# Roboy/gym-roboy

Hardware: AMD Instinct MI355X
Metric: env-steps/sec, MsjRobot (3-DOF/8-tendon) batched rollout (higher is better)
Workload: dtype f32

## Files before the change

### gym_roboy_amd/csrc/gen_msj_baked.cpp

```cpp
#include <cstdio>
#include <string>

#include "msj_build.hpp"

extern "C" int rb_gen_msj_baked(const rb_robot_desc *d, double step_size, int nsub, const char *path) {
    rb::MsjConst<float, 8> c;
    std::string err;
    const int rc = rb::msj_build<float, 8>(d, step_size, nsub, &c, err);
    if (rc) return rc;
    FILE *f = std::fopen(path, "w");
    if (!f) return RB_EINVAL;
    std::fprintf(f, "// msj_baked.hpp - GENERATED by gen_msj_baked.cpp (tools/gen_msj_baked.py) from\n"
                    "// gym_roboy_amd/envs/robots/data/msj_platform.json: MsjRobot's closed-form constants as literals.\n"
                    "// Do not edit; regenerate.  Hex float literals: exact.\n#pragma once\n#include \"msj_math.hpp\"\n\nnamespace rbk {\n"
                    "#define RB_MSJ_BAKED_TABLE {{ \\\n");
    for (int k = 0; k < 8; ++k) {
        const auto &t = c.ten[k];
        std::fprintf(f, "  {{%af,%af,%af},{%af,%af,%af},{%af,%af,%af},%af,%af,%af,%af,%af,{0.0f,0.0f}}, \\\n", t.A[0], t.A[1], t.A[2],
                     t.Bv[0], t.Bv[1], t.Bv[2], t.B2[0], t.B2[1], t.B2[2], t.ab2, t.il0s, t.elcs, t.ksg, t.fmaxv);
    }
    std::fprintf(f, " }, {%af,%af,%af,%af,%af,%af}, {%af,%af,%af}, {%af,%af,%af}, \\\n", c.IO[0], c.IO[1], c.IO[2], c.IO[3], c.IO[4],
                 c.IO[5], c.mc[0], c.mc[1], c.mc[2], c.g[0], c.g[1], c.g[2]);
    std::fprintf(f, " {%af,%af,%af},{%af,%af,%af},{%af,%af,%af},{%af,%af,%af},{%af,%af,%af}, \\\n", c.arm[0], c.arm[1], c.arm[2],
                 c.damp[0], c.damp[1], c.damp[2], c.qlo[0], c.qlo[1], c.qlo[2], c.qhi[0], c.qhi[1], c.qhi[2], c.qdmax[0],
                 c.qdmax[1], c.qdmax[2]);
    std::fprintf(f, " %af,%af,%af,%af,%af,%af,%af,%af, %d,%d,%d}\n", c.kps, c.pe_k2s, c.inv_pe_den, c.fv_c1l, c.fv_c2l, c.fv_c2s,
                 c.fv_k, c.h, c.nsub, c.simple, c.nt);
    std::fprintf(f, "#if defined(__HIPCC__)\n__device__ constexpr rb::MsjConst<float, 8> BAKED = RB_MSJ_BAKED_TABLE;\n#endif\n"
                    "constexpr rb::MsjConst<float, 8> BAKED_HOST = RB_MSJ_BAKED_TABLE;\n}  // namespace rbk\n");
    std::fclose(f);
    return RB_OK;
}
```

### gym_roboy_amd/csrc/msj_baked.hpp

```cpp
#pragma once
#include "msj_math.hpp"

namespace rbk {
#define RB_MSJ_BAKED_TABLE {{ \
  {{0x1.5784fcp-4f,0x1.be2b16p-5f,-0x1.47ae14p-6f},{0x1.179142p-7f,0x1.48d0b8p-5f,0x1.b03512p-5f},{-0x1.dce646p-6f,-0x1.187458p-3f,-0x1.70a3d8p-3f},0x1.7f62b6p-6f,0x1.9090f6p+3f,-0x1.a30d8ap+0f,0x1.2c24dap+2f,0x1.99674ep+5f,{0.0f,0.0f}}, \
  {{0x1.be2b16p-5f,0x1.5784fcp-4f,-0x1.47ae14p-6f},{0x1.48d0b8p-5f,0x1.179142p-7f,0x1.b03512p-5f},{-0x1.187458p-3f,-0x1.dce646p-6f,-0x1.70a3d8p-3f},0x1.7f62b6p-6f,0x1.9090f6p+3f,-0x1.a30d8ap+0f,0x1.2c24dap+2f,0x1.99674ep+5f,{0.0f,0.0f}}, \
  {{-0x1.be2b16p-5f,0x1.5784fcp-4f,-0x1.47ae14p-6f},{-0x1.48d0b8p-5f,0x1.179142p-7f,0x1.b03512p-5f},{0x1.187458p-3f,-0x1.dce646p-6f,-0x1.70a3d8p-3f},0x1.7f62b6p-6f,0x1.9090f6p+3f,-0x1.a30d8ap+0f,0x1.2c24dap+2f,0x1.4785d8p+3f,{0.0f,0.0f}}, \
  {{-0x1.5784fcp-4f,0x1.be2b16p-5f,-0x1.47ae14p-6f},{-0x1.179142p-7f,0x1.48d0b8p-5f,0x1.b03512p-5f},{0x1.dce646p-6f,-0x1.187458p-3f,-0x1.70a3d8p-3f},0x1.7f62b6p-6f,0x1.9090f6p+3f,-0x1.a30d8ap+0f,0x1.2c24dap+2f,0x1.4785d8p+3f,{0.0f,0.0f}}, \
  {{-0x1.5784fcp-4f,-0x1.be2b16p-5f,-0x1.47ae14p-6f},{-0x1.179142p-7f,-0x1.48d0b8p-5f,0x1.b03512p-5f},{0x1.dce646p-6f,0x1.187458p-3f,-0x1.70a3d8p-3f},0x1.7f62b6p-6f,0x1.9090f6p+3f,-0x1.a30d8ap+0f,0x1.2c24dap+2f,0x1.4785d8p+3f,{0.0f,0.0f}}, \
  {{-0x1.be2b16p-5f,-0x1.5784fcp-4f,-0x1.47ae14p-6f},{-0x1.48d0b8p-5f,-0x1.179142p-7f,0x1.b03512p-5f},{0x1.187458p-3f,0x1.dce646p-6f,-0x1.70a3d8p-3f},0x1.7f62b6p-6f,0x1.9090f6p+3f,-0x1.a30d8ap+0f,0x1.2c24dap+2f,0x1.4785d8p+3f,{0.0f,0.0f}}, \
  {{0x1.be2b16p-5f,-0x1.5784fcp-4f,-0x1.47ae14p-6f},{0x1.48d0b8p-5f,-0x1.179142p-7f,0x1.b03512p-5f},{-0x1.187458p-3f,0x1.dce646p-6f,-0x1.70a3d8p-3f},0x1.7f62b6p-6f,0x1.9090f6p+3f,-0x1.a30d8ap+0f,0x1.2c24dap+2f,0x1.99674ep+5f,{0.0f,0.0f}}, \
  {{0x1.5784fcp-4f,-0x1.be2b16p-5f,-0x1.47ae14p-6f},{0x1.179142p-7f,-0x1.48d0b8p-5f,0x1.b03512p-5f},{-0x1.dce646p-6f,0x1.187458p-3f,-0x1.70a3d8p-3f},0x1.7f62b6p-6f,0x1.9090f6p+3f,-0x1.a30d8ap+0f,0x1.2c24dap+2f,0x1.99674ep+5f,{0.0f,0.0f}}, \
 }, {0x1.3a92a4p-10f,0x1.3a92a4p-10f,0x1.0624dep-11f,0x0p+0f,0x0p+0f,0x0p+0f}, {0x0p+0f,0x0p+0f,0x1.eb851ep-7f}, {0x0p+0f,0x0p+0f,-0x1.39eb86p+3f}, \
 {0x1.99999ap-3f,0x1.99999ap-3f,0x1.99999ap-3f},{0x1.99999ap-1f,0x1.99999ap-1f,0x1.99999ap-1f},{-0x1.ccccccp-2f,-0x1.ccccccp-2f,-0x1.333334p-1f},{0x1.ccccccp-2f,0x1.ccccccp-2f,0x1.333334p-1f},{0x1.0c1524p-1f,0x1.0c1524p-1f,0x1.0c1524p-1f}, \
 0x1.df8d2cp+1f,0x1.cd3b24p+1f,0x1.31aea4p-6f,0x1.ep+3f,0x1.4p+3f,-0x1p+2f,0x1.4p+2f,0x1.99999ap-4f, 1,1,8}
#if defined(__HIPCC__)
__device__ constexpr rb::MsjConst<float, 8> BAKED = RB_MSJ_BAKED_TABLE;
#endif
constexpr rb::MsjConst<float, 8> BAKED_HOST = RB_MSJ_BAKED_TABLE;
}
```

### gym_roboy_amd/csrc/msj_build.hpp

```cpp
#pragma once
#include <cmath>
#include <string>

#include "../../include/roboy_sim.h"
#include "msj_math.hpp"

namespace rb {

inline bool msj_class(const rb_robot_desc *d, std::string &why) {
    if (d->n_q != 3) { why = "n_q != 3"; return false; }
    for (int i = 0; i < 3; ++i) {
        if (d->parent[i] != i - 1) { why = "joints are not a serial chain"; return false; }
        for (int a = 0; a < 3; ++a) {
            if (d->origin[3 * i + a] != 0.0) { why = "joint origins are not co-located at the base origin"; return false; }
            if (std::fabs(d->axis[3 * i + a] - (a == i ? 1.0 : 0.0)) > 1e-12) { why = "joint axes are not x, y, z"; return false; }
        }
    }
    for (int i = 0; i < 2; ++i) {
        if (d->mass[i] != 0.0) { why = "virtual links 0/1 carry mass"; return false; }
        for (int a = 0; a < 6; ++a)
            if (d->inertia[6 * i + a] != 0.0) { why = "virtual links 0/1 carry inertia"; return false; }
    }
    for (int k = 0; k < d->n_t; ++k) {
        const int v0 = d->vp_offset[k], v1 = d->vp_offset[k + 1];
        if (v1 - v0 < 2) { why = "tendon with fewer than two via-points"; return false; }
        bool on_body = false;
        for (int v = v0; v < v1; ++v) {
            const int link = d->vp_link[v];
            if (link != -1 && link != 2) { why = "via-point on a virtual link"; return false; }
            if (link == 2) on_body = true;
            else if (on_body) { why = "tendon returns from the body to the base"; return false; }
        }
        if (d->vp_link[v0] != -1 || !on_body) { why = "tendon does not run base -> body"; return false; }
    }
    return true;
}

template <typename T, int NT>
int msj_build(const rb_robot_desc *d, double step_size, int nsub, MsjConst<T, NT> *out, std::string &err,
              bool exact = true) {
    if (!msj_class(d, err)) return RB_EUNSUPPORTED;
    if (exact ? d->n_t != NT : (d->n_t < 1 || d->n_t > NT)) {
        err = "tendon count does not match this kernel instance"; return RB_EUNSUPPORTED;
    }
    MsjConst<T, NT> &c = *out;
    const double log2e = 1.4426950408889634;
    const double sc = std::sqrt(log2e) / d->fl_width;
    auto seglen = [&](int va, int vb) {
        double s = 0.0;
        for (int a = 0; a < 3; ++a) { const double t = d->vp_pos[3 * vb + a] - d->vp_pos[3 * va + a]; s += t * t; }
        return std::sqrt(s);
    };
    for (int k = 0; k < d->n_t; ++k) {
        const int v0 = d->vp_offset[k], v1 = d->vp_offset[k + 1];
        int vb = v0;
        while (d->vp_link[vb] == -1) ++vb;
        const int va = vb - 1;
        double lc = 0.0;
        for (int v = v0; v + 1 < v1; ++v)
            if (v != va) lc += seglen(v, v + 1);
        const double moving0 = seglen(va, vb);
        if (moving0 < 1e-6) { err = "degenerate tendon segment"; return RB_EINVAL; }
        const double l0 = lc + moving0;
        MsjTendon<T> &t = c.ten[k];
        const double vl0 = d->v_max * l0;
        for (int a = 0; a < 3; ++a) { t.A[a] = T(d->vp_pos[3 * va + a]); t.Bv[a] = T(d->vp_pos[3 * vb + a] / vl0); }
        double ab2 = 0.0;
        for (int a = 0; a < 3; ++a) ab2 += d->vp_pos[3 * va + a] * d->vp_pos[3 * va + a] + d->vp_pos[3 * vb + a] * d->vp_pos[3 * vb + a];
        for (int a = 0; a < 3; ++a) t.B2[a] = T(-2.0 * d->vp_pos[3 * vb + a]);
        t.ab2 = T(ab2); t.il0s = T(sc / l0); t.elcs = T(sc * (lc / l0 - 1.0)); t.ksg = T(d->kp * d->setpoint_scale / l0);
        t.fmaxv = T(d->f_max[k] * vl0);
        t.pad[0] = t.pad[1] = T(0);
    }
    for (int k = d->n_t; k < NT; ++k) {
        MsjTendon<T> &t = c.ten[k];
        t.A[0] = T(1); t.A[1] = T(0); t.A[2] = T(0); t.Bv[0] = T(0); t.Bv[1] = T(0); t.Bv[2] = T(1);
        t.B2[0] = T(0); t.B2[1] = T(0); t.B2[2] = T(-2);
        t.ab2 = T(2); t.il0s = T(sc); t.elcs = T(-sc); t.ksg = T(0); t.fmaxv = T(0);
        t.pad[0] = t.pad[1] = T(0);
    }
    c.nt = d->n_t;
    const double m = d->mass[2];
    const double *cm = d->com + 6, *ic = d->inertia + 12;
    const double c2 = cm[0] * cm[0] + cm[1] * cm[1] + cm[2] * cm[2];
    c.IO[0] = T(ic[0] + m * (c2 - cm[0] * cm[0]));
    c.IO[1] = T(ic[1] + m * (c2 - cm[1] * cm[1]));
    c.IO[2] = T(ic[2] + m * (c2 - cm[2] * cm[2]));
    c.IO[3] = T(ic[3] - m * cm[0] * cm[1]);
    c.IO[4] = T(ic[4] - m * cm[0] * cm[2]);
    c.IO[5] = T(ic[5] - m * cm[1] * cm[2]);
    for (int a = 0; a < 3; ++a) {
        c.mc[a] = T(m * cm[a]);
        c.g[a] = T(d->gravity[a]);
        c.arm[a] = T(d->armature[a]); c.damp[a] = T(d->damping[a]);
        c.qlo[a] = T(d->q_lo[a]); c.qhi[a] = T(d->q_hi[a]); c.qdmax[a] = T(d->qd_max[a]);
    }
    c.kps = T(d->kp / sc);
    c.pe_k2s = T(log2e * d->kpe / (d->e0 * sc));
    c.inv_pe_den = T(1.0 / (std::exp(d->kpe) - 1.0));
    const double slope0 = 1.0 + 1.0 / d->fv_a;
    const double c2l = slope0 / (d->fv_n - 1.0);
    c.fv_c2s = T(-1.0 / d->fv_a);
    c.fv_k = T(1.0 + 1.0 / d->fv_a);
    c.fv_c1l = T(d->fv_n * c2l); c.fv_c2l = T(c2l);
    c.h = T(step_size / nsub); c.nsub = nsub;
    c.simple = (ic[3] == 0.0 && ic[4] == 0.0 && ic[5] == 0.0 && cm[0] == 0.0 && cm[1] == 0.0 &&
                d->gravity[0] == 0.0 && d->gravity[1] == 0.0) ? 1 : 0;
    return RB_OK;
}

template <typename T>
void msj_tendon_units(const rb_robot_desc *d, TendonUnits<T> *out, int nt_max) {
// ... 57 lines not shown
```

### gym_roboy_amd/csrc/msj_jit.hpp

```cpp
#pragma once
#include <dlfcn.h>
#include <hip/hip_runtime.h>
#include <hip/hiprtc.h>

#include <fcntl.h>
#include <sys/stat.h>
#include <unistd.h>

#include <atomic>
#include <cstdint>
#include <cstdio>
#include <cstdlib>
#include <cstring>
#include <string>
#include <vector>

#include "msj_math.hpp"

namespace rbj {

struct Module {
    hipModule_t mod = nullptr;
    hipFunction_t step[2] = {nullptr, nullptr};
    hipFunction_t env[2] = {nullptr, nullptr};
// ... 11 lines not shown
    decltype(&hiprtcGetCode) code = nullptr;
    decltype(&hiprtcDestroyProgram) destroy = nullptr;
    decltype(&hiprtcVersion) version = nullptr;
    bool ok = false;
};

inline const Rtc &rtc() {
    static Rtc r = [] {
        Rtc x;
        void *h = dlopen("libhiprtc.so", RTLD_NOW | RTLD_GLOBAL);
        if (!h) h = dlopen("/opt/rocm/lib/libhiprtc.so", RTLD_NOW | RTLD_GLOBAL);
        if (!h) return x;
#define RBJ_SYM(field, name) x.field = reinterpret_cast<decltype(x.field)>(dlsym(h, name))
        RBJ_SYM(create, "hiprtcCreateProgram"); RBJ_SYM(add_name, "hiprtcAddNameExpression");
        RBJ_SYM(compile, "hiprtcCompileProgram"); RBJ_SYM(log_size, "hiprtcGetProgramLogSize");
        RBJ_SYM(log, "hiprtcGetProgramLog"); RBJ_SYM(lowered, "hiprtcGetLoweredName");
        RBJ_SYM(code_size, "hiprtcGetCodeSize"); RBJ_SYM(code, "hiprtcGetCode"); RBJ_SYM(destroy, "hiprtcDestroyProgram");
        RBJ_SYM(version, "hiprtcVersion");
#undef RBJ_SYM
        x.ok = x.create && x.add_name && x.compile && x.log_size && x.log && x.lowered && x.code_size && x.code && x.destroy;
        return x;
    }();
    return r;
}

inline std::string table_text(const rb::MsjConst<float, 8> &c) {
    std::string s = "{{";
    char buf[64];
    auto f = [&](float v) { std::snprintf(buf, sizeof buf, "%af,", double(v)); s += buf; };
    for (int k = 0; k < 8; ++k) {
        const auto &t = c.ten[k];
        s += "{{"; f(t.A[0]); f(t.A[1]); f(t.A[2]); s += "},{"; f(t.Bv[0]); f(t.Bv[1]); f(t.Bv[2]); s += "},{";
        f(t.B2[0]); f(t.B2[1]); f(t.B2[2]); s += "},";
        f(t.ab2); f(t.il0s); f(t.elcs); f(t.ksg); f(t.fmaxv); s += "{0.0f,0.0f}},";
    }
    s += "},{"; for (int a = 0; a < 6; ++a) f(c.IO[a]);
    s += "},{"; for (int a = 0; a < 3; ++a) f(c.mc[a]);
    s += "},{"; for (int a = 0; a < 3; ++a) f(c.g[a]);
    s += "},{"; for (int a = 0; a < 3; ++a) f(c.arm[a]);
    s += "},{"; for (int a = 0; a < 3; ++a) f(c.damp[a]);
    s += "},{"; for (int a = 0; a < 3; ++a) f(c.qlo[a]);
    s += "},{"; for (int a = 0; a < 3; ++a) f(c.qhi[a]);
    s += "},{"; for (int a = 0; a < 3; ++a) f(c.qdmax[a]);
    s += "},"; f(c.kps); f(c.pe_k2s); f(c.inv_pe_den); f(c.fv_c1l); f(c.fv_c2l); f(c.fv_c2s); f(c.fv_k); f(c.h);
    s += std::to_string(c.nsub) + "," + std::to_string(c.simple) + "," + std::to_string(c.nt) + "}";
    return s;
}

inline std::string library_dir() {
    Dl_info info;
    if (!dladdr(reinterpret_cast<const void *>(&library_dir), &info) || !info.dli_fname) return ".";
    std::string p = info.dli_fname;
    const size_t k = p.rfind('/');
    return k == std::string::npos ? "." : p.substr(0, k);
}

inline bool enabled() {
    const char *e = std::getenv("ROBOY_SIM_JIT");
    return !(e && e[0] == '0');
}

struct CacheStats { std::atomic<long long> hits{0}, compiles{0}, stores{0}; };
inline CacheStats &cache_stats() { static CacheStats s; return s; }

inline std::string cache_dir() {
    const char *e = std::getenv("ROBOY_SIM_JIT_CACHE");
    std::string d;
// ... 176 lines not shown
```

### gym_roboy_amd/csrc/msj_kernels.hpp

```cpp
#pragma once
#include "rtc_compat.hpp"
#include "msj_math.hpp"
#include "philox.hpp"
#include "env_common.hpp"

#if defined(RB_JIT_TABLE)
namespace rbk { __device__ constexpr rb::MsjConst<float, 8> BAKED = RB_JIT_TABLE; }
#else
#include "msj_baked.hpp"
#endif

namespace rbk {

using rbe::EnvParams;
using rbe::GoalBox;
using rbe::goal_value;
using rbe::mul_then_add;

constexpr int NT8 = 8;
constexpr int RS = rb::MsjModel<float, 8>::RS;
using Const8 = rb::MsjConst<float, NT8>;
constexpr int NTX = 16;
using ConstX = rb::MsjConst<float, NTX>;


template <bool BK, typename CONST>
__device__ __forceinline__ const CONST &robot_consts(const CONST &kernarg) {
    if constexpr (BK) return rbk::BAKED; else return kernarg;
}

struct SpLds {
    const float *col;
    int stride;
    __device__ __forceinline__ float operator()(int k) const { return col[k * stride]; }
};

template <int KEEP>
struct SpSplit {
    const float *reg;
    const float *col;
    int stride;
    __device__ __forceinline__ float operator()(int k) const { return k < KEEP ? reg[k] : col[(k - KEEP) * stride]; }
};

struct Scale8 { float v[NT8]; };

template <int INTEG, int BLOCK, int UNROLL, bool BK = false>
__global__ void __launch_bounds__(BLOCK)
msj_step_env_per_lane(const Const8 c_arg, float *__restrict__ q, float *__restrict__ qd,
                      uint32_t *__restrict__ feas, const float *__restrict__ act, const Scale8 us, long n, long cnt) {
    const Const8 &c = robot_consts<BK>(c_arg);
    const long i = long(blockIdx.x) * BLOCK + threadIdx.x;
    if (i >= cnt) return;
    float qq[3], vv[3], sp[NT8];
    const float4 a0 = reinterpret_cast<const float4 *>(act)[2 * i];
    const float4 a1 = reinterpret_cast<const float4 *>(act)[2 * i + 1];
#pragma unroll
    for (int j = 0; j < 3; ++j) { qq[j] = q[j * n + i]; vv[j] = qd[j * n + i]; }
    const float a[NT8] = {a0.x, a0.y, a0.z, a0.w, a1.x, a1.y, a1.z, a1.w};
#pragma unroll
    for (int k = 0; k < NT8; ++k) sp[k] = a[k] * us.v[k];
    bool ok;
// ... 15 lines not shown

__device__ __forceinline__ __amdgpu_buffer_rsrc_t wg_rsrc(const void *base, int bytes) {
    return __builtin_amdgcn_make_buffer_rsrc(const_cast<void *>(base), 0, bytes, 0x00020000);
}

template <int INTEG, int BLOCK, bool BK = false>
__global__ void __launch_bounds__(BLOCK)
msj_step_env_per_lane_rs(const Const8 c_arg, float *__restrict__ q, float *__restrict__ qd,
                         uint32_t *__restrict__ feas, const float *__restrict__ act, const Scale8 us, long n, long cnt) {
    const Const8 &c = robot_consts<BK>(c_arg);
    const long env0 = long(blockIdx.x) * BLOCK;
    const long left = cnt - env0;
    const int live = int(left < BLOCK ? left : BLOCK);
    const int le = int(threadIdx.x);
    if (le >= live) return;
    const int off = le * 4;
    float qq[3], vv[3], u[NT8];
    const __amdgpu_buffer_rsrc_t ra = wg_rsrc(act + env0 * NT8, live * NT8 * 4);
    typedef float f4 __attribute__((ext_vector_type(4)));
    const f4 a0 = __builtin_bit_cast(f4, __builtin_amdgcn_raw_buffer_load_b128(ra, off * NT8, 0, 0));
    const f4 a1 = __builtin_bit_cast(f4, __builtin_amdgcn_raw_buffer_load_b128(ra, off * NT8 + 16, 0, 0));
#pragma unroll
    for (int j = 0; j < 3; ++j) {
        qq[j] = __uint_as_float(__builtin_amdgcn_raw_buffer_load_b32(wg_rsrc(q + j * n + env0, live * 4), off, 0, 0));
        vv[j] = __uint_as_float(__builtin_amdgcn_raw_buffer_load_b32(wg_rsrc(qd + j * n + env0, live * 4), off, 0, 0));
    }
    const float a[NT8] = {a0.x, a0.y, a0.z, a0.w, a1.x, a1.y, a1.z, a1.w};
#pragma unroll
    for (int k = 0; k < NT8; ++k) u[k] = a[k] * us.v[k];
    constexpr int KEEP = NT8 - 2;
    __shared__ float lds_u[NT8 - KEEP][BLOCK];
#pragma unroll
    for (int k = KEEP; k < NT8; ++k) lds_u[k - KEEP][le] = u[k];
    const bool ok = rb::MsjModel<float, NT8>::template step_rs_paired<INTEG>(c, qq, vv, SpSplit<KEEP>{u, &lds_u[0][le], BLOCK});
#pragma unroll
    for (int j = 0; j < 3; ++j) {
        __builtin_amdgcn_raw_buffer_store_b32(__float_as_uint(qq[j]), wg_rsrc(q + j * n + env0, live * 4), off, 0, 0);
        __builtin_amdgcn_raw_buffer_store_b32(__float_as_uint(vv[j]), wg_rsrc(qd + j * n + env0, live * 4), off, 0, 0);
    }
    __builtin_amdgcn_raw_buffer_store_b32(ok ? 1u : 0u, wg_rsrc(feas + env0, live * 4), off, 0, 0);
}


struct PairMap { int a[4], d[4]; };
struct Scale4 { float v[4]; };

template <int CTRL>
__device__ __forceinline__ float rbk_dpp(float v) {
    return __int_as_float(__builtin_amdgcn_update_dpp(0, __float_as_int(v), CTRL, 0xF, 0xF, true));
}

template <int MIRROR>
struct AccelMirrorHalf {
    const Const8 &c;
    const float *u;
    __device__ __forceinline__ void operator()(const float q[3], const float qd[3], float qdd[3]) const {
        using M = rb::MsjModel<float, NT8>;
        const M::Frame f = M::frame(q, qd);
        float tx, ty, tz;
        M::half_torque(c, f, u, tx, ty, tz);
        M::template mirror_combine<MIRROR>(tx, ty, tz, rbk_dpp<0xB1>(tx), rbk_dpp<0xB1>(ty), rbk_dpp<0xB1>(tz));
        M::rigid_body(c, f, qd, tx, ty, tz, qdd);
    }
};

template <int INTEG, int BLOCK, int MIRROR, bool BK = false>
__global__ void __launch_bounds__(BLOCK)
// ... 26 lines not shown
    for (int j = 0; j < 3; ++j) {
        __builtin_amdgcn_raw_buffer_store_b32(__float_as_uint(qq[j]), wg_rsrc(q + j * n + env0, live * 4), soff, 0, 0);
        __builtin_amdgcn_raw_buffer_store_b32(__float_as_uint(vv[j]), wg_rsrc(qd + j * n + env0, live * 4), soff, 0, 0);
    }
    __builtin_amdgcn_raw_buffer_store_b32(ok ? 1u : 0u, wg_rsrc(feas + env0, live * 4), soff, 0, 0);
}


template <int INTEG, int BLOCK, int UNROLL, bool BK = false>
__global__ void __launch_bounds__(BLOCK)
msj_rollout_fused(const Const8 c_arg, float *__restrict__ q, float *__restrict__ qd, uint32_t *__restrict__ feas,
                  const float *__restrict__ act_ring, int ring, int n_steps, const Scale8 us, long n) {
    const Const8 &c = robot_consts<BK>(c_arg);
    const long i = long(blockIdx.x) * BLOCK + threadIdx.x;
    if (i >= n) return;
    float qq[3], vv[3];
#pragma unroll
    for (int j = 0; j < 3; ++j) { qq[j] = q[j * n + i]; vv[j] = qd[j * n + i]; }
    bool ok = true;
    const float4 *rec = reinterpret_cast<const float4 *>(act_ring) + 2 * i;
    float4 a0 = rec[0], a1 = rec[1];
    __shared__ float lds_sp[UNROLL >= NT8 ? 1 : NT8][BLOCK];
    int slab = 0;
    for (int t = 0; t < n_steps; ++t) {
        const float a[NT8] = {a0.x, a0.y, a0.z, a0.w, a1.x, a1.y, a1.z, a1.w};
        float sp[NT8];
#pragma unroll
        for (int k = 0; k < NT8; ++k) sp[k] = a[k] * us.v[k];
        if (t + 1 < n_steps) {
            slab = slab + 1 == ring ? 0 : slab + 1;
            const float4 *nx = rec + long(slab) * 2 * n;
            a0 = nx[0]; a1 = nx[1];
        }
        if (UNROLL == RS) {
            ok = rb::MsjModel<float, NT8>::template step_rs<INTEG>(c, qq, vv, sp);
        } else if (UNROLL >= NT8) {
            ok = rb::MsjModel<float, NT8>::template step_sp<INTEG, UNROLL>(c, qq, vv, rb::SpArray<float, NT8>{sp});
        } else {
#pragma unroll
            for (int k = 0; k < NT8; ++k) lds_sp[k][threadIdx.x] = sp[k];
            ok = rb::MsjModel<float, NT8>::template step_sp<INTEG, UNROLL>(c, qq, vv, SpLds{&lds_sp[0][threadIdx.x], BLOCK});
        }
    }
#pragma unroll
    for (int j = 0; j < 3; ++j) { q[j * n + i] = qq[j]; qd[j * n + i] = vv[j]; }
    feas[i] = ok ? 1u : 0u;
}



__device__ __forceinline__ void draw_goal3(const float (&lo)[3], const float (&hi)[3], uint64_t seed, uint64_t gid, uint32_t draw, float g[3]) {
    const rb::Philox4 r = rb::philox_draw(seed, gid, draw, rb::STREAM_GOALS, 0u);
#pragma unroll
    for (int j = 0; j < 3; ++j) g[j] = goal_value(lo[j], hi[j], r.v[j]);
}
__device__ __forceinline__ void draw_goal3(const GoalBox &box, uint64_t seed, uint64_t gid, uint32_t draw, float g[3]) {
    const float lo[3] = {box.lo[0], box.lo[1], box.lo[2]}, hi[3] = {box.hi[0], box.hi[1], box.hi[2]};
    draw_goal3(lo, hi, seed, gid, draw, g);
}

struct MsjEnvArgs {
    EnvParams e;
    float box_lo[3], box_hi[3];
    float *q, *qd;
    uint32_t *feas;
    float *goal;
    uint32_t *step_num;
// ... 107 lines not shown
     \
    const float *__restrict__ q = a.q, *__restrict__ qd = a.qd, *__restrict__ goal = a.goal, *__restrict__ act = a.act;             \
    const long n = a.n, cnt = a.cnt;                                                                                                \
    const float slope = a.e.slope, act_hi = a.e.act_hi;                                                                             \
    const CONST &c = robot_consts<BK>(c_arg);                                                                                       \
    const long i = long(blockIdx.x) * BLOCK + threadIdx.x;                                                                          \
    if (i >= cnt) return;                                                                                                           \
    float qq[3], vv[3], gg[3];                                                                                                      \
    _Pragma("unroll")                                                                                                               \
    for (int j = 0; j < 3; ++j) { qq[j] = q[j * n + i]; vv[j] = qd[j * n + i]; gg[j] = goal[j * n + i]; }                           \
     \
    decltype((OX).applied(a.step_num, act, i, 0)) ap{};         \
    auto rescale = [&](float x) { return ap.rest ? 0.0f : rbe::action_setpoint(slope, x, act_hi); };                                \
    bool ok;                                                                                                                        \
    HeldOffsets held{nullptr, nullptr, 1};                                                                                          \
    constexpr bool IN_LDS = UNROLL != RS && UNROLL < NT8;                                                                           \
    float sp[NT8];                                                                                                                  \
    if constexpr (UNROLL == 0) {                                                                                                    \
        __shared__ float lds_sp[NTX][BLOCK];                                                                                        \
        const int nt = c.nt;                                                                                                        \
        ap = (OX).applied(a.step_num, act, i, nt);                                                                                  \
        const float *row = ap.row;                                                                                                  \
        for (int k = 0; k < nt; ++k) lds_sp[k][threadIdx.x] = rescale(row[k]) * c.ten[k].ksg;                                       \
        ok = rb::MsjModel<float, NTX>::template step_sp<INTEG, 0>(c, qq, vv, SpLds{&lds_sp[0][threadIdx.x], BLOCK});                \
        held = HeldOffsets{&lds_sp[0][threadIdx.x], nullptr, BLOCK};                                                                \
    } else {                                                                                                                        \
    held.u = sp;                                                                                                                    \
    ap = (OX).applied(a.step_num, act, i, NT8);                                                                                     \
    const float4 a0 = reinterpret_cast<const float4 *>(ap.row)[0];                                                                  \
    const float4 a1 = reinterpret_cast<const float4 *>(ap.row)[1];                                                                  \
    const float av[NT8] = {a0.x, a0.y, a0.z, a0.w, a1.x, a1.y, a1.z, a1.w};                                                         \
    _Pragma("unroll")                                                                                                               \
    for (int k = 0; k < NT8; ++k) sp[k] = rescale(av[k]) * c.ten[k].ksg;                                                            \
    if (UNROLL == RS) {                                                                                                             \
        ok = rb::MsjModel<float, NT8>::template step_rs<INTEG>(c, qq, vv, sp);                                                      \
    } else if (UNROLL >= NT8) {                                                                                                     \
        ok = rb::MsjModel<float, NT8>::template step_sp<INTEG, UNROLL>(c, qq, vv, rb::SpArray<float, NT8>{sp});                     \
    } else {                                                                                                                        \
         \
         \
        __shared__ float lds_sp[NT8][BLOCK];                                                                                        \
    _Pragma("unroll")                                                                                                               \
        for (int k = 0; k < NT8; ++k) lds_sp[k][threadIdx.x] = sp[k];                                                               \
        ok = rb::MsjModel<float, NT8>::template step_sp<INTEG, UNROLL>(c, qq, vv, SpLds{&lds_sp[0][threadIdx.x], BLOCK});           \
        held = HeldOffsets{&lds_sp[0][threadIdx.x], nullptr, BLOCK};                                                                \
    }                                                                                                                               \
    }                                                                                                                               \
    if constexpr (BK) {                                                                                                             \
        env_account(&a, i, qq, vv, gg, ok, (OX).done_hook(&a, NoDoneHook{}), (OX).template policy<IN_LDS>(&a, ap, c, held, i));     \
    } else {                                                                                                                        \
        const msj_env_kernarg_ptr la = late_env_args(msj_env_args_offset(int(sizeof(CONST))));                                      \
        env_account(la, i, qq, vv, gg, ok, (OX).done_hook(la, NoDoneHook{}), (OX).template policy<IN_LDS>(la, ap, c, held, i));     \
    }
template <int INTEG, int BLOCK, int UNROLL, typename CONST = Const8, bool BK = false>
__global__ void __launch_bounds__(BLOCK)
msj_env_step_kernel(const CONST c_arg, const MsjEnvArgs a) {
    RB_MSJ_ENV_STEP_BODY(NoObsExt{})
}


template <int INTEG, int BLOCK, int MIRROR, bool BK = false>
__global__ void __launch_bounds__(BLOCK)
msj_env_step_mirror_pairs(const Const8 c_arg, const PairMap pm, const MsjEnvArgs a) {
    const float *__restrict__ q = a.q, *__restrict__ qd = a.qd, *__restrict__ goal = a.goal, *__restrict__ act = a.act;
    const long n = a.n, cnt = a.cnt;
    const float slope = a.e.slope, act_hi = a.e.act_hi;
    const Const8 &c = robot_consts<BK>(c_arg);
// ... 34 lines not shown
```

### gym_roboy_amd/csrc/msj_math.hpp

```cpp
#pragma once
#include "rtc_compat.hpp"

#if defined(__HIPCC__)
#define RB_HD __host__ __device__ __forceinline__
#else
#define RB_HD inline
#endif


namespace rb {

template <typename T> struct Fast;
template <> struct Fast<double> {
    static RB_HD void sincos(double x, double &s, double &c) { s = ::sin(x); c = ::cos(x); }
    static RB_HD double exp(double x) { return ::exp(x); }
    static RB_HD double exp2(double x) { return ::exp2(x); }
    static RB_HD double rsqrt(double x) { return 1.0 / ::sqrt(x); }
    static RB_HD double rcp(double x) { return 1.0 / x; }
};
template <> struct Fast<float> {
    static RB_HD void sincos(float x, float &s, float &c) {
#if defined(__HIP_DEVICE_COMPILE__)
        s = __sinf(x); c = __cosf(x);
#else
        s = ::sinf(x); c = ::cosf(x);
#endif
    }
    static RB_HD float exp(float x) {
#if defined(__HIP_DEVICE_COMPILE__)
        return __expf(x);
#else
        return ::expf(x);
#endif
    }
    static RB_HD float exp2(float x) {
#if defined(__HIP_DEVICE_COMPILE__)
        return __builtin_amdgcn_exp2f(x);
#else
        return ::exp2f(x);
#endif
    }
    static RB_HD float rsqrt(float x) {
#if defined(__HIP_DEVICE_COMPILE__)
        return __builtin_amdgcn_rsqf(x);
#else
        return 1.0f / ::sqrtf(x);
#endif
    }
    static RB_HD float rcp(float x) {
#if defined(__HIP_DEVICE_COMPILE__)
        return __builtin_amdgcn_rcpf(x);
#else
        return 1.0f / x;
#endif
    }
};

template <typename T> RB_HD T tmin(T a, T b) {
#if defined(__HIP_DEVICE_COMPILE__)
    if constexpr (std::is_same<T, float>::value) return __builtin_fminf(a, b);
#endif
    return a < b ? a : b;
}
template <typename T> RB_HD T tmax(T a, T b) {
#if defined(__HIP_DEVICE_COMPILE__)
    if constexpr (std::is_same<T, float>::value) return __builtin_fmaxf(a, b);
#endif
    return a > b ? a : b;
}
template <typename T> RB_HD T tclamp(T x, T lo, T hi) {
#if defined(__HIP_DEVICE_COMPILE__)
    if constexpr (std::is_same<T, float>::value) return __builtin_amdgcn_fmed3f(x, lo, hi);
#endif
    return tmin(tmax(x, lo), hi);
}

template <typename T>
struct alignas(64) MsjTendon {
    T A[3];
    T Bv[3];
    T B2[3];
    T ab2;
    T il0s;
    T elcs;
    T ksg;
    T fmaxv;
    T pad[2];
};

template <typename T>
struct TendonUnits {
    T lc;
    T vl0;
    T fmax;
    T pad;
};

template <typename T>
struct TendonReading { T length, rate, activation, force; };

template <typename T, int NT>
struct MsjConst {
    MsjTendon<T> ten[NT];
    T IO[6];
    T mc[3];
    T g[3];
    T arm[3], damp[3], qlo[3], qhi[3], qdmax[3];
    T kps;
    T pe_k2s;
    T inv_pe_den;
    T fv_c1l, fv_c2l;
    T fv_c2s;
    T fv_k;
    T h;
    int32_t nsub;
    int32_t simple;
    int32_t nt;
};

template <typename T, int NT>
// ... 146 lines not shown
            m01 = s2 * a0x + c2 * a0y;
            m02 = a0z;
            m11 = s2 * a1x + c2 * a1y + c.arm[1];
            m12 = a1z;
            m22 = Izz + c.arm[2];
            const T hx = a0x * qd[0] + a1x * qd[1] + Ixz * qd[2];
            const T hy = a0y * qd[0] + a1y * qd[1] + Iyz * qd[2];
            const T hz = a0z * qd[0] + a1z * qd[1] + Izz * qd[2];
            const T nx = Ixx * bx + Ixy * by + Ixz * bz + (f.wy * hz - f.wz * hy);
            const T ny = Ixy * bx + Iyy * by + Iyz * bz + (f.wz * hx - f.wx * hz);
            const T nz = Ixz * bx + Iyz * by + Izz * bz + (f.wx * hy - f.wy * hx);
            const T gx = r00 * c.g[0] + f.r10 * c.g[1] + f.r20 * c.g[2];
            const T gy = r01 * c.g[0] + f.r11 * c.g[1] + f.r21 * c.g[2];
            const T gz = r02 * c.g[0] + f.r12 * c.g[1] + f.r22 * c.g[2];
            vx = tx + (bmass(bp, c.mc[1]) * gz - bmass(bp, c.mc[2]) * gy) - nx;
            vy = ty + (bmass(bp, c.mc[2]) * gx - bmass(bp, c.mc[0]) * gz) - ny;
            vz = tz + (bmass(bp, c.mc[0]) * gy - bmass(bp, c.mc[1]) * gx) - nz;
        }
        const T t0 = r00 * vx + r01 * vy + r02 * vz - bdamp(bp, 0, c.damp[0]) * qd[0];
        const T t1 = s2 * vx + c2 * vy - bdamp(bp, 1, c.damp[1]) * qd[1];
        const T t2 = vz - bdamp(bp, 2, c.damp[2]) * qd[2];
        const T k00 = m11 * m22 - m12 * m12;
        const T k01 = m02 * m12 - m01 * m22;
        const T k02 = m01 * m12 - m02 * m11;
        const T k11 = m00 * m22 - m02 * m02;
        const T k12 = m01 * m02 - m00 * m12;
        const T k22 = m00 * m11 - m01 * m01;
        const T idet = Fast<T>::rcp(m00 * k00 + m01 * k01 + m02 * k02);
        qdd[0] = (k00 * t0 + k01 * t1 + k02 * t2) * idet;
        qdd[1] = (k01 * t0 + k11 * t1 + k12 * t2) * idet;
        qdd[2] = (k02 * t0 + k12 * t1 + k22 * t2) * idet;
    }

    template <int UNROLL, typename SP>
    struct AccelAllTendons {
        const C &c;
        const SP &sp;
        RB_HD void operator()(const T q[3], const T qd[3], T qdd[3]) const {
            const Frame f = frame(q, qd);
            T tx = T(0), ty = T(0), tz = T(0);
            if (UNROLL == 0) {
#pragma unroll 1
                for (int k = 0; k < c.nt; ++k) tendon(c, f, c.ten[k], sp(k), tx, ty, tz);
            } else {
                constexpr int U = UNROLL > 0 ? UNROLL : 1;
#pragma unroll U
                for (int k = 0; k < NT; ++k) tendon(c, f, c.ten[k], sp(k), tx, ty, tz);
            }
            rigid_body(c, f, qd, tx, ty, tz, qdd);
        }
    };

    template <int MIRROR> static RB_HD T mirror_sign(int j) { return (j == 2 || j == MIRROR) ? T(-1) : T(1); }
    static RB_HD void half_torque(const C &c, const Frame &f, const T u[4], T &tx, T &ty, T &tz) {
        tx = T(0); ty = T(0); tz = T(0);
#pragma unroll
        for (int k = 0; k < 4; ++k) {
            tendon(c, f, c.ten[k], u[k], tx, ty, tz);
#if defined(__HIP_DEVICE_COMPILE__)
            __builtin_amdgcn_sched_barrier(0);
#endif
        }
    }
    template <int MIRROR>
    static RB_HD void mirror_combine(T &tx, T &ty, T &tz, T px, T py, T pz) {
        tx = MIRROR == 0 ? tx - px : tx + px;
// ... 154 lines not shown
        const Routing ra = routing(f, ta);
        pin();
        const T ia = Fast<T>::rsqrt(ra.d2);
        const Routing rb_ = routing(f, tb);
        pin();
        const T ib = Fast<T>::rsqrt(rb_.d2);
        const Strain sa = strain(c, f, ta, ra, ia);
        pin();
        const Hill ha = hill(c, sa, ua);
        const Strain sb = strain(c, f, tb, rb_, ib);
        pin();
        torque(c, ta, ra, ia, sa, ha, tx, ty, tz);
        const Hill hb = hill(c, sb, ub);
        pin();
        torque(c, tb, rb_, ib, sb, hb, tx, ty, tz);
        pin();
    }
    template <typename SP>
    struct AccelPaired {
        const C &c;
        const SP &sp;
        RB_HD void operator()(const T q[3], const T qd[3], T qdd[3]) const {
            static_assert(NT % 2 == 0, "tendons in pairs");
            const Frame f = frame(q, qd);
            T tx = T(0), ty = T(0), tz = T(0);
#pragma unroll
            for (int k = 0; k < NT; k += 2) {
                const T ua = sp(k), ub = sp(k + 1);
                tendon_pair(c, f, c.ten[k], c.ten[k + 1], ua, ub, tx, ty, tz);
            }
            rigid_body(c, f, qd, tx, ty, tz, qdd);
        }
    };
    static constexpr int RS = 9;
    template <int INTEG>
    static RB_HD bool step_rs(const C &c, T q[3], T qd[3], const T u[NT]) {
        return integrate_acc<INTEG>(c, q, qd, AccelPinned{c, u});
    }

    template <int INTEG, typename SP>
    static RB_HD bool step_rs_paired(const C &c, T q[3], T qd[3], const SP &sp) {
        return integrate_acc<INTEG>(c, q, qd, AccelPaired<SP>{c, sp});
    }

    template <int INTEG, int UNROLL, typename SP>
    static RB_HD bool step_sp(const C &c, T q[3], T qd[3], const SP &sp) {
        return integrate<INTEG>(c, q, qd, AccelAllTendons<UNROLL, SP>{c, sp});
    }

    template <int INTEG, int UNROLL = NT>
    static RB_HD bool step(const C &c, T q[3], T qd[3], const T sp[NT]) {
        T u[NT];
#pragma unroll
        for (int k = 0; k < NT; ++k) u[k] = prescale(c, k, sp[k]);
        const SpArray<T, NT> src{u};
        return step_sp<INTEG, UNROLL>(c, q, qd, src);
    }
};

}
```

Measured before the change: 20.32 billion.

## Fold fmax into exponent constants and specialize axisymmetric rigid-body solve for baked MSJ

Adds two per-tendon constants, log2(fmax) and a prescaled passive-elastic coefficient, in the old padding slots. This lets the force-length exp2 absorb the fmax multiply through an fma, and lets the passive force be computed without separate scaling. When the baked robot has equal x/y inertia and a simple body, a specialized rigid-body solve is used that drops zero terms and solves a 2x2 plus a scalar system instead of the full 3x3. The path is only enabled for baked constants with INTEG==1 and BLOCK==256, and it relies on fmax being non-negative and on exact constant folding.

```diff
diff --git a/gym_roboy_amd/csrc/gen_msj_baked.cpp b/gym_roboy_amd/csrc/gen_msj_baked.cpp
--- a/gym_roboy_amd/csrc/gen_msj_baked.cpp
+++ b/gym_roboy_amd/csrc/gen_msj_baked.cpp
@@ -16,8 +16,8 @@
                     "#define RB_MSJ_BAKED_TABLE {{ \\\n");
     for (int k = 0; k < 8; ++k) {
         const auto &t = c.ten[k];
-        std::fprintf(f, "  {{%af,%af,%af},{%af,%af,%af},{%af,%af,%af},%af,%af,%af,%af,%af,{0.0f,0.0f}}, \\\n", t.A[0], t.A[1], t.A[2],
-                     t.Bv[0], t.Bv[1], t.Bv[2], t.B2[0], t.B2[1], t.B2[2], t.ab2, t.il0s, t.elcs, t.ksg, t.fmaxv);
+        std::fprintf(f, "  {{%af,%af,%af},{%af,%af,%af},{%af,%af,%af},%af,%af,%af,%af,%af,%af,%af}, \\\n", t.A[0], t.A[1], t.A[2],
+                     t.Bv[0], t.Bv[1], t.Bv[2], t.B2[0], t.B2[1], t.B2[2], t.ab2, t.il0s, t.elcs, t.ksg, t.fmaxv, t.lfmax, t.pecf);
     }
     std::fprintf(f, " }, {%af,%af,%af,%af,%af,%af}, {%af,%af,%af}, {%af,%af,%af}, \\\n", c.IO[0], c.IO[1], c.IO[2], c.IO[3], c.IO[4],
                  c.IO[5], c.mc[0], c.mc[1], c.mc[2], c.g[0], c.g[1], c.g[2]);
diff --git a/gym_roboy_amd/csrc/msj_baked.hpp b/gym_roboy_amd/csrc/msj_baked.hpp
--- a/gym_roboy_amd/csrc/msj_baked.hpp
+++ b/gym_roboy_amd/csrc/msj_baked.hpp
@@ -3,14 +3,14 @@
 
 namespace rbk {
 #define RB_MSJ_BAKED_TABLE {{ \
-  {{0x1.5784fcp-4f,0x1.be2b16p-5f,-0x1.47ae14p-6f},{0x1.179142p-7f,0x1.48d0b8p-5f,0x1.b03512p-5f},{-0x1.dce646p-6f,-0x1.187458p-3f,-0x1.70a3d8p-3f},0x1.7f62b6p-6f,0x1.9090f6p+3f,-0x1.a30d8ap+0f,0x1.2c24dap+2f,0x1.99674ep+5f,{0.0f,0.0f}}, \
-  {{0x1.be2b16p-5f,0x1.5784fcp-4f,-0x1.47ae14p-6f},{0x1.48d0b8p-5f,0x1.179142p-7f,0x1.b03512p-5f},{-0x1.187458p-3f,-0x1.dce646p-6f,-0x1.70a3d8p-3f},0x1.7f62b6p-6f,0x1.9090f6p+3f,-0x1.a30d8ap+0f,0x1.2c24dap+2f,0x1.99674ep+5f,{0.0f,0.0f}}, \
-  {{-0x1.be2b16p-5f,0x1.5784fcp-4f,-0x1.47ae14p-6f},{-0x1.48d0b8p-5f,0x1.179142p-7f,0x1.b03512p-5f},{0x1.187458p-3f,-0x1.dce646p-6f,-0x1.70a3d8p-3f},0x1.7f62b6p-6f,0x1.9090f6p+3f,-0x1.a30d8ap+0f,0x1.2c24dap+2f,0x1.4785d8p+3f,{0.0f,0.0f}}, \
-  {{-0x1.5784fcp-4f,0x1.be2b16p-5f,-0x1.47ae14p-6f},{-0x1.179142p-7f,0x1.48d0b8p-5f,0x1.b03512p-5f},{0x1.dce646p-6f,-0x1.187458p-3f,-0x1.70a3d8p-3f},0x1.7f62b6p-6f,0x1.9090f6p+3f,-0x1.a30d8ap+0f,0x1.2c24dap+2f,0x1.4785d8p+3f,{0.0f,0.0f}}, \
-  {{-0x1.5784fcp-4f,-0x1.be2b16p-5f,-0x1.47ae14p-6f},{-0x1.179142p-7f,-0x1.48d0b8p-5f,0x1.b03512p-5f},{0x1.dce646p-6f,0x1.187458p-3f,-0x1.70a3d8p-3f},0x1.7f62b6p-6f,0x1.9090f6p+3f,-0x1.a30d8ap+0f,0x1.2c24dap+2f,0x1.4785d8p+3f,{0.0f,0.0f}}, \
-  {{-0x1.be2b16p-5f,-0x1.5784fcp-4f,-0x1.47ae14p-6f},{-0x1.48d0b8p-5f,-0x1.179142p-7f,0x1.b03512p-5f},{0x1.187458p-3f,0x1.dce646p-6f,-0x1.70a3d8p-3f},0x1.7f62b6p-6f,0x1.9090f6p+3f,-0x1.a30d8ap+0f,0x1.2c24dap+2f,0x1.4785d8p+3f,{0.0f,0.0f}}, \
-  {{0x1.be2b16p-5f,-0x1.5784fcp-4f,-0x1.47ae14p-6f},{0x1.48d0b8p-5f,-0x1.179142p-7f,0x1.b03512p-5f},{-0x1.187458p-3f,0x1.dce646p-6f,-0x1.70a3d8p-3f},0x1.7f62b6p-6f,0x1.9090f6p+3f,-0x1.a30d8ap+0f,0x1.2c24dap+2f,0x1.99674ep+5f,{0.0f,0.0f}}, \
-  {{0x1.5784fcp-4f,-0x1.be2b16p-5f,-0x1.47ae14p-6f},{0x1.179142p-7f,-0x1.48d0b8p-5f,0x1.b03512p-5f},{-0x1.dce646p-6f,0x1.187458p-3f,-0x1.70a3d8p-3f},0x1.7f62b6p-6f,0x1.9090f6p+3f,-0x1.a30d8ap+0f,0x1.2c24dap+2f,0x1.99674ep+5f,{0.0f,0.0f}}, \
+  {{0x1.5784fcp-4f,0x1.be2b16p-5f,-0x1.47ae14p-6f},{0x1.179142p-7f,0x1.48d0b8p-5f,0x1.b03512p-5f},{-0x1.dce646p-6f,-0x1.187458p-3f,-0x1.70a3d8p-3f},0x1.7f62b6p-6f,0x1.9090f6p+3f,-0x1.a30d8ap+0f,0x1.2c24dap+2f,0x1.99674ep+5f,0x1.6b5a3p+2f,0x1.e8db5ep-1f}, \
+  {{0x1.be2b16p-5f,0x1.5784fcp-4f,-0x1.47ae14p-6f},{0x1.48d0b8p-5f,0x1.179142p-7f,0x1.b03512p-5f},{-0x1.187458p-3f,-0x1.dce646p-6f,-0x1.70a3d8p-3f},0x1.7f62b6p-6f,0x1.9090f6p+3f,-0x1.a30d8ap+0f,0x1.2c24dap+2f,0x1.99674ep+5f,0x1.6b5a3p+2f,0x1.e8db5ep-1f}, \
+  {{-0x1.be2b16p-5f,0x1.5784fcp-4f,-0x1.47ae14p-6f},{-0x1.48d0b8p-5f,0x1.179142p-7f,0x1.b03512p-5f},{0x1.187458p-3f,-0x1.dce646p-6f,-0x1.70a3d8p-3f},0x1.7f62b6p-6f,0x1.9090f6p+3f,-0x1.a30d8ap+0f,0x1.2c24dap+2f,0x1.4785d8p+3f,0x1.ad7f7p+1f,0x1.8715e6p-3f}, \
+  {{-0x1.5784fcp-4f,0x1.be2b16p-5f,-0x1.47ae14p-6f},{-0x1.179142p-7f,0x1.48d0b8p-5f,0x1.b03512p-5f},{0x1.dce646p-6f,-0x1.187458p-3f,-0x1.70a3d8p-3f},0x1.7f62b6p-6f,0x1.9090f6p+3f,-0x1.a30d8ap+0f,0x1.2c24dap+2f,0x1.4785d8p+3f,0x1.ad7f7p+1f,0x1.8715e6p-3f}, \
+  {{-0x1.5784fcp-4f,-0x1.be2b16p-5f,-0x1.47ae14p-6f},{-0x1.179142p-7f,-0x1.48d0b8p-5f,0x1.b03512p-5f},{0x1.dce646p-6f,0x1.187458p-3f,-0x1.70a3d8p-3f},0x1.7f62b6p-6f,0x1.9090f6p+3f,-0x1.a30d8ap+0f,0x1.2c24dap+2f,0x1.4785d8p+3f,0x1.ad7f7p+1f,0x1.8715e6p-3f}, \
+  {{-0x1.be2b16p-5f,-0x1.5784fcp-4f,-0x1.47ae14p-6f},{-0x1.48d0b8p-5f,-0x1.179142p-7f,0x1.b03512p-5f},{0x1.187458p-3f,0x1.dce646p-6f,-0x1.70a3d8p-3f},0x1.7f62b6p-6f,0x1.9090f6p+3f,-0x1.a30d8ap+0f,0x1.2c24dap+2f,0x1.4785d8p+3f,0x1.ad7f7p+1f,0x1.8715e6p-3f}, \
+  {{0x1.be2b16p-5f,-0x1.5784fcp-4f,-0x1.47ae14p-6f},{0x1.48d0b8p-5f,-0x1.179142p-7f,0x1.b03512p-5f},{-0x1.187458p-3f,0x1.dce646p-6f,-0x1.70a3d8p-3f},0x1.7f62b6p-6f,0x1.9090f6p+3f,-0x1.a30d8ap+0f,0x1.2c24dap+2f,0x1.99674ep+5f,0x1.6b5a3p+2f,0x1.e8db5ep-1f}, \
+  {{0x1.5784fcp-4f,-0x1.be2b16p-5f,-0x1.47ae14p-6f},{0x1.179142p-7f,-0x1.48d0b8p-5f,0x1.b03512p-5f},{-0x1.dce646p-6f,0x1.187458p-3f,-0x1.70a3d8p-3f},0x1.7f62b6p-6f,0x1.9090f6p+3f,-0x1.a30d8ap+0f,0x1.2c24dap+2f,0x1.99674ep+5f,0x1.6b5a3p+2f,0x1.e8db5ep-1f}, \
  }, {0x1.3a92a4p-10f,0x1.3a92a4p-10f,0x1.0624dep-11f,0x0p+0f,0x0p+0f,0x0p+0f}, {0x0p+0f,0x0p+0f,0x1.eb851ep-7f}, {0x0p+0f,0x0p+0f,-0x1.39eb86p+3f}, \
  {0x1.99999ap-3f,0x1.99999ap-3f,0x1.99999ap-3f},{0x1.99999ap-1f,0x1.99999ap-1f,0x1.99999ap-1f},{-0x1.ccccccp-2f,-0x1.ccccccp-2f,-0x1.333334p-1f},{0x1.ccccccp-2f,0x1.ccccccp-2f,0x1.333334p-1f},{0x1.0c1524p-1f,0x1.0c1524p-1f,0x1.0c1524p-1f}, \
  0x1.df8d2cp+1f,0x1.cd3b24p+1f,0x1.31aea4p-6f,0x1.ep+3f,0x1.4p+3f,-0x1p+2f,0x1.4p+2f,0x1.99999ap-4f, 1,1,8}
diff --git a/gym_roboy_amd/csrc/msj_build.hpp b/gym_roboy_amd/csrc/msj_build.hpp
--- a/gym_roboy_amd/csrc/msj_build.hpp
+++ b/gym_roboy_amd/csrc/msj_build.hpp
@@ -51,6 +51,8 @@
         for (int a = 0; a < 3; ++a) { const double t = d->vp_pos[3 * vb + a] - d->vp_pos[3 * va + a]; s += t * t; }
         return std::sqrt(s);
     };
+    auto as_stored = [](double x) { return std::is_same<T, float>::value ? double(float(x)) : x; };
+    const double ipd = as_stored(1.0 / (std::exp(d->kpe) - 1.0));
     for (int k = 0; k < d->n_t; ++k) {
         const int v0 = d->vp_offset[k], v1 = d->vp_offset[k + 1];
         int vb = v0;
@@ -70,14 +72,16 @@
         for (int a = 0; a < 3; ++a) t.B2[a] = T(-2.0 * d->vp_pos[3 * vb + a]);
         t.ab2 = T(ab2); t.il0s = T(sc / l0); t.elcs = T(sc * (lc / l0 - 1.0)); t.ksg = T(d->kp * d->setpoint_scale / l0);
         t.fmaxv = T(d->f_max[k] * vl0);
-        t.pad[0] = t.pad[1] = T(0);
+        const double fm = as_stored(d->f_max[k] * vl0);
+        t.lfmax = fm > 0.0 ? T(std::log2(fm)) : T(-2000);
+        t.pecf = T(ipd * fm);
     }
     for (int k = d->n_t; k < NT; ++k) {
         MsjTendon<T> &t = c.ten[k];
         t.A[0] = T(1); t.A[1] = T(0); t.A[2] = T(0); t.Bv[0] = T(0); t.Bv[1] = T(0); t.Bv[2] = T(1);
         t.B2[0] = T(0); t.B2[1] = T(0); t.B2[2] = T(-2);
         t.ab2 = T(2); t.il0s = T(sc); t.elcs = T(-sc); t.ksg = T(0); t.fmaxv = T(0);
-        t.pad[0] = t.pad[1] = T(0);
+        t.lfmax = T(-2000); t.pecf = T(0);
     }
     c.nt = d->n_t;
     const double m = d->mass[2];
diff --git a/gym_roboy_amd/csrc/msj_jit.hpp b/gym_roboy_amd/csrc/msj_jit.hpp
--- a/gym_roboy_amd/csrc/msj_jit.hpp
+++ b/gym_roboy_amd/csrc/msj_jit.hpp
@@ -67,7 +67,7 @@
         const auto &t = c.ten[k];
         s += "{{"; f(t.A[0]); f(t.A[1]); f(t.A[2]); s += "},{"; f(t.Bv[0]); f(t.Bv[1]); f(t.Bv[2]); s += "},{";
         f(t.B2[0]); f(t.B2[1]); f(t.B2[2]); s += "},";
-        f(t.ab2); f(t.il0s); f(t.elcs); f(t.ksg); f(t.fmaxv); s += "{0.0f,0.0f}},";
+        f(t.ab2); f(t.il0s); f(t.elcs); f(t.ksg); f(t.fmaxv); f(t.lfmax); f(t.pecf); s += "},";
     }
     s += "},{"; for (int a = 0; a < 6; ++a) f(c.IO[a]);
     s += "},{"; for (int a = 0; a < 3; ++a) f(c.mc[a]);
diff --git a/gym_roboy_amd/csrc/msj_kernels.hpp b/gym_roboy_amd/csrc/msj_kernels.hpp
--- a/gym_roboy_amd/csrc/msj_kernels.hpp
+++ b/gym_roboy_amd/csrc/msj_kernels.hpp
@@ -28,6 +28,10 @@
 __device__ __forceinline__ const CONST &robot_consts(const CONST &kernarg) {
     if constexpr (BK) return rbk::BAKED; else return kernarg;
 }
+
+template <int INTEG, int BLOCK, bool BK>
+constexpr bool FOLDED_ACCEL = BK && INTEG == 1 && BLOCK == 256 && rb::MsjModel<float, NT8>::foldable(rbk::BAKED);
+constexpr bool BAKED_AXISYM = rb::MsjModel<float, NT8>::axisymmetric(rbk::BAKED);
 
 struct SpLds {
     const float *col;
@@ -109,7 +113,11 @@
     __shared__ float lds_u[NT8 - KEEP][BLOCK];
 #pragma unroll
     for (int k = KEEP; k < NT8; ++k) lds_u[k - KEEP][le] = u[k];
-    const bool ok = rb::MsjModel<float, NT8>::template step_rs_paired<INTEG>(c, qq, vv, SpSplit<KEEP>{u, &lds_u[0][le], BLOCK});
+    bool ok;
+    if constexpr (FOLDED_ACCEL<INTEG, BLOCK, BK>)
+        ok = rb::MsjModel<float, NT8>::template step_rs_folded<INTEG, BAKED_AXISYM>(c, qq, vv, SpSplit<KEEP>{u, &lds_u[0][le], BLOCK});
+    else
+        ok = rb::MsjModel<float, NT8>::template step_rs_paired<INTEG>(c, qq, vv, SpSplit<KEEP>{u, &lds_u[0][le], BLOCK});
 #pragma unroll
     for (int j = 0; j < 3; ++j) {
         __builtin_amdgcn_raw_buffer_store_b32(__float_as_uint(qq[j]), wg_rsrc(q + j * n + env0, live * 4), off, 0, 0);
@@ -202,7 +210,9 @@
             const float4 *nx = rec + long(slab) * 2 * n;
             a0 = nx[0]; a1 = nx[1];
         }
-        if (UNROLL == RS) {
+        if constexpr (UNROLL == RS && FOLDED_ACCEL<INTEG, BLOCK, BK>) {
+            ok = rb::MsjModel<float, NT8>::template step_rs_folded<INTEG, BAKED_AXISYM>(c, qq, vv, rb::SpArray<float, NT8>{sp});
+        } else if (UNROLL == RS) {
             ok = rb::MsjModel<float, NT8>::template step_rs<INTEG>(c, qq, vv, sp);
         } else if (UNROLL >= NT8) {
             ok = rb::MsjModel<float, NT8>::template step_sp<INTEG, UNROLL>(c, qq, vv, rb::SpArray<float, NT8>{sp});
@@ -376,7 +386,9 @@
     const float av[NT8] = {a0.x, a0.y, a0.z, a0.w, a1.x, a1.y, a1.z, a1.w};                                                         \
     _Pragma("unroll")                                                                                                               \
     for (int k = 0; k < NT8; ++k) sp[k] = rescale(av[k]) * c.ten[k].ksg;                                                            \
-    if (UNROLL == RS) {                                                                                                             \
+    if constexpr (UNROLL == RS && FOLDED_ACCEL<INTEG, BLOCK, BK>) {               \
+        ok = rb::MsjModel<float, NT8>::template step_rs_folded<INTEG, BAKED_AXISYM>(c, qq, vv, rb::SpArray<float, NT8>{sp});        \
+    } else if (UNROLL == RS) {                                                                                                      \
         ok = rb::MsjModel<float, NT8>::template step_rs<INTEG>(c, qq, vv, sp);                                                      \
     } else if (UNROLL >= NT8) {                                                                                                     \
         ok = rb::MsjModel<float, NT8>::template step_sp<INTEG, UNROLL>(c, qq, vv, rb::SpArray<float, NT8>{sp});                     \
diff --git a/gym_roboy_amd/csrc/msj_math.hpp b/gym_roboy_amd/csrc/msj_math.hpp
--- a/gym_roboy_amd/csrc/msj_math.hpp
+++ b/gym_roboy_amd/csrc/msj_math.hpp
@@ -17,6 +17,7 @@
     static RB_HD double exp2(double x) { return ::exp2(x); }
     static RB_HD double rsqrt(double x) { return 1.0 / ::sqrt(x); }
     static RB_HD double rcp(double x) { return 1.0 / x; }
+    static RB_HD double fma(double a, double b, double c) { return __builtin_fma(a, b, c); }
 };
 template <> struct Fast<float> {
     static RB_HD void sincos(float x, float &s, float &c) {
@@ -54,6 +55,7 @@
         return 1.0f / x;
 #endif
     }
+    static RB_HD float fma(float a, float b, float c) { return __builtin_fmaf(a, b, c); }
 };
 
 template <typename T> RB_HD T tmin(T a, T b) {
@@ -85,7 +87,8 @@
     T elcs;
     T ksg;
     T fmaxv;
-    T pad[2];
+    T lfmax;
+    T pecf;
 };
 
 template <typename T>
@@ -298,6 +301,37 @@
         qdd[2] = (k02 * t0 + k12 * t1 + k22 * t2) * idet;
     }
 
+    static constexpr RB_HD bool axisymmetric(const C &c) { return c.simple != 0 && c.IO[0] == c.IO[1]; }
+    static RB_HD void rigid_body_axisym(const C &c, const Frame &f, const T qd[3], T tx, T ty, T tz, T qdd[3]) {
+        const T r00 = f.r00, r01 = f.r01, r02 = f.r02, s2 = f.s2, c2 = f.c2;
+        const T I = c.IO[0], Izz = c.IO[2];
+        const T z0x = -f.s1 * c2 * qd[1] - f.c1 * s2 * qd[2];
+        const T z0y = f.s1 * s2 * qd[1] - f.c1 * c2 * qd[2];
+        const T z0z = f.c1 * qd[1];
+        const T bx = z0x * qd[0] + c2 * qd[2] * qd[1];
+        const T by = z0y * qd[0] - s2 * qd[2] * qd[1];
+        const T bz = z0z * qd[0];
+        const T m00 = (Izz - I) * (f.s1 * f.s1) + (I + c.arm[0]);
+        const T m02 = Izz * f.s1;
+        const T m22 = Izz + c.arm[2];
+        const T im11 = T(1) / (I + c.arm[1]);
+        const T g = (Izz - I) * f.wz;
+        const T nx = I * bx + f.wy * g;
+        const T ny = I * by - f.wx * g;
+        const T nz = Izz * bz;
+        const T k = c.mc[2] * c.g[2];
+        const T vx = tx - k * f.r21 - nx;
+        const T vy = ty + k * f.r20 - ny;
+        const T vz = tz - nz;
+        const T t0 = r00 * vx + r01 * vy + r02 * vz - c.damp[0] * qd[0];
+        const T t1 = s2 * vx + c2 * vy - c.damp[1] * qd[1];
+        const T t2 = vz - c.damp[2] * qd[2];
+        const T idet = Fast<T>::rcp(m00 * m22 - m02 * m02);
+        qdd[0] = (m22 * t0 - m02 * t2) * idet;
+        qdd[1] = t1 * im11;
+        qdd[2] = (m00 * t2 - m02 * t0) * idet;
+    }
+
     template <int UNROLL, typename SP>
     struct AccelAllTendons {
         const C &c;
@@ -518,6 +552,64 @@
             rigid_body(c, f, qd, tx, ty, tz, qdd);
         }
     };
+    static RB_HD Strain strain_folded(const C &c, const Frame &f, const MsjTendon<T> &t, const Routing &r, T inv) {
+        Strain s;
+        s.v = (f.wx * r.mx + f.wy * r.my + f.wz * r.mz) * inv;
+        s.es = (r.d2 * inv) * t.il0s + t.elcs;
+        s.fl = Fast<T>::exp2(Fast<T>::fma(-s.es, s.es, t.lfmax));
+        s.pe = Fast<T>::exp2(c.pe_k2s * s.es);
+        return s;
+    }
+    static RB_HD void torque_folded(const MsjTendon<T> &t, const Routing &r, T inv, const Strain &s, const Hill &h, T &tx, T &ty, T &tz) {
+        const T fpe = tmax(s.pe * t.pecf - t.pecf, T(0));
+        const T Fs = inv * (h.afn * h.rden + fpe);
+        tx -= Fs * r.mx; ty -= Fs * r.my; tz -= Fs * r.mz;
+    }
+    static constexpr RB_HD bool foldable(const C &c) {
+        for (int k = 0; k < NT; ++k)
+            if (!(c.ten[k].fmaxv >= T(0))) return false;
+        return true;
+    }
+    static RB_HD void tendon_pair_folded(const C &c, const Frame &f, const MsjTendon<T> &ta, const MsjTendon<T> &tb, T ua, T ub,
+                                         T &tx, T &ty, T &tz) {
+        const Routing ra = routing(f, ta);
+        pin();
+        const T ia = Fast<T>::rsqrt(ra.d2);
+        const Routing rb_ = routing(f, tb);
+        pin();
+        const T ib = Fast<T>::rsqrt(rb_.d2);
+        const Strain sa = strain_folded(c, f, ta, ra, ia);
+        pin();
+        const Hill ha = hill(c, sa, ua);
+        const Strain sb = strain_folded(c, f, tb, rb_, ib);
+        pin();
+        torque_folded(ta, ra, ia, sa, ha, tx, ty, tz);
+        const Hill hb = hill(c, sb, ub);
+        pin();
+        torque_folded(tb, rb_, ib, sb, hb, tx, ty, tz);
+        pin();
+    }
+    template <typename SP, bool AXISYM>
+    struct AccelFolded {
+        const C &c;
+        const SP &sp;
+        template <int K>
+        RB_HD void pairs_from(const Frame &f, T &tx, T &ty, T &tz) const {
+            if constexpr (K < NT) {
+                const T ua = sp(K), ub = sp(K + 1);
+                tendon_pair_folded(c, f, c.ten[K], c.ten[K + 1], ua, ub, tx, ty, tz);
+                pairs_from<K + 2>(f, tx, ty, tz);
+            }
+        }
+        RB_HD void operator()(const T q[3], const T qd[3], T qdd[3]) const {
+            static_assert(NT % 2 == 0, "tendons in pairs");
+            const Frame f = frame(q, qd);
+            T tx = T(0), ty = T(0), tz = T(0);
+            pairs_from<0>(f, tx, ty, tz);
+            if constexpr (AXISYM) rigid_body_axisym(c, f, qd, tx, ty, tz, qdd);
+            else rigid_body(c, f, qd, tx, ty, tz, qdd);
+        }
+    };
     static constexpr int RS = 9;
     template <int INTEG>
     static RB_HD bool step_rs(const C &c, T q[3], T qd[3], const T u[NT]) {
@@ -529,6 +621,11 @@
         return integrate_acc<INTEG>(c, q, qd, AccelPaired<SP>{c, sp});
     }
 
+    template <int INTEG, bool AXISYM, typename SP>
+    static RB_HD bool step_rs_folded(const C &c, T q[3], T qd[3], const SP &sp) {
+        return integrate_acc<INTEG>(c, q, qd, AccelFolded<SP, AXISYM>{c, sp});
+    }
+
     template <int INTEG, int UNROLL, typename SP>
     static RB_HD bool step_sp(const C &c, T q[3], T qd[3], const SP &sp) {
         return integrate<INTEG>(c, q, qd, AccelAllTendons<UNROLL, SP>{c, sp});
```

After: 21.77 billion, median of 6. 1.07x the previous value.
